# omkhairate/MetalPathtracer

Measured on AMD Instinct MI355X. Metric: Mrays/s at 1920x1080x256spp on scene.xml, higher is better.
Workload: dtype f32; 1 GPU; scene.xml 1920x1080 x 256 spp per step, depth 8 (181 steps timed); prims=4971, bvh_nodes=2289, bvh_builder=device, rng=philox4x32-10 (pixel,sample,bounce), pipeline=wave-local wavefront, reference-order walk, parallelism=8x8-tile interleave over 1 rank(s), rays=161154900585

## Files before the change

### metalpathtracer_amd/csrc/mpt_device.h

```cpp
#pragma once
#include <hip/hip_runtime.h>
#include <stdint.h>

#define MPT_WAVE 64
#define MPT_NSHARD 16
#define MPT_NGROUP 8
#define MPT_NONE 0xFFFFFFFFu

struct F3 {
    float x, y, z;
};
__device__ __forceinline__ F3 f3(float x, float y, float z) { return F3{x, y, z}; }
__device__ __forceinline__ F3 operator+(F3 a, F3 b) { return F3{a.x + b.x, a.y + b.y, a.z + b.z}; }
__device__ __forceinline__ F3 operator-(F3 a, F3 b) { return F3{a.x - b.x, a.y - b.y, a.z - b.z}; }
__device__ __forceinline__ F3 operator*(F3 a, float s) { return F3{a.x * s, a.y * s, a.z * s}; }
__device__ __forceinline__ F3 operator*(float s, F3 a) { return F3{s * a.x, s * a.y, s * a.z}; }
__device__ __forceinline__ F3 operator-(F3 a) { return F3{-a.x, -a.y, -a.z}; }
__device__ __forceinline__ float dot3(F3 a, F3 b) { return a.x * b.x + a.y * b.y + a.z * b.z; }
__device__ __forceinline__ F3 cross3(F3 a, F3 b) {
    return F3{a.y * b.z - a.z * b.y, a.z * b.x - a.x * b.z, a.x * b.y - a.y * b.x};
}
#ifndef MPT_FAST_RCP
#define MPT_FAST_RCP 3
#endif
#define MPT_RCP_LO 1.1754943508222875e-38f
#define MPT_RCP_HI 8.5070591730234616e+37f
__device__ __forceinline__ float rcp_chain(float x) {
    float r = __builtin_amdgcn_rcpf(x);
    const float e0 = fmaf(-x, r, 1.0f);
    r = fmaf(e0, r, r);
    float q = r;
    const float e1 = fmaf(-x, q, 1.0f);
    q = fmaf(e1, r, q);
    const float e2 = fmaf(-x, q, 1.0f);
    return fmaf(e2, r, q);
}
__device__ __forceinline__ bool rcp_chain_exact(float x) { return fabsf(x) >= MPT_RCP_LO && fabsf(x) <= MPT_RCP_HI; }
__device__ __forceinline__ float mpt_rcp(float x) {
#if MPT_FAST_RCP == 2
    return rcp_chain(x);
#elif MPT_FAST_RCP == 3
    if (__builtin_expect(__ballot(!rcp_chain_exact(x)) == 0ull, 1)) return rcp_chain(x);
    return 1.0f / x;
#elif MPT_FAST_RCP == 1
    float r = rcp_chain(x);
    if (__builtin_expect(!rcp_chain_exact(x), 0)) r = 1.0f / x;
    return r;
#else
    return 1.0f / x;
#endif
}
__device__ __forceinline__ void mpt_rcp3(float x, float y, float z, float& ix, float& iy, float& iz) {
#if MPT_FAST_RCP == 3
    if (__builtin_expect(__ballot(!(rcp_chain_exact(x) && rcp_chain_exact(y) && rcp_chain_exact(z))) == 0ull, 1)) {
        ix = rcp_chain(x);
        iy = rcp_chain(y);
        iz = rcp_chain(z);
        return;
    }
    ix = 1.0f / x;
    iy = 1.0f / y;
    iz = 1.0f / z;
#else
    ix = mpt_rcp(x);
    iy = mpt_rcp(y);
    iz = mpt_rcp(z);
#endif
}
__device__ __forceinline__ F3 normalize3(F3 a) {
    float inv = mpt_rcp(sqrtf(dot3(a, a)));
    return a * inv;
}
#ifndef MPT_LEAN_SQRT
#define MPT_LEAN_SQRT 1
#endif
#define MPT_SQRT_LO 0x1p-96f
#define MPT_NORM_HI 0x1p126f
__device__ __forceinline__ float sqrt_core(float x) {
    const float s = __builtin_amdgcn_sqrtf(x);
    const float lo = __uint_as_float(__float_as_uint(s) - 1u), hi = __uint_as_float(__float_as_uint(s) + 1u);
    const float vlo = fmaf(-lo, s, x), vhi = fmaf(-hi, s, x);
    float r = vlo <= 0.0f ? lo : s;
    r = vhi > 0.0f ? hi : r;
    return r;
}
__device__ __forceinline__ bool sqrt_core_exact(float x) { return x >= MPT_SQRT_LO && x < INFINITY; }
__device__ __forceinline__ bool norm_core_exact(float l2) { return l2 >= MPT_SQRT_LO && l2 <= MPT_NORM_HI; }
__device__ __forceinline__ float inv_len_core(float l2) { return rcp_chain(sqrt_core(l2)); }
template <bool LEAN>
__device__ __forceinline__ F3 normalize3(F3 a) {
    if (LEAN && MPT_LEAN_SQRT) {
        const float l2 = dot3(a, a);
        if (__builtin_expect(__ballot(!norm_core_exact(l2)) == 0ull, 1)) return a * inv_len_core(l2);
        return a * mpt_rcp(sqrtf(l2));
    }
    return normalize3(a);
}
#ifndef MPT_LEAN_CDIV
#define MPT_LEAN_CDIV 1
#endif
__device__ __forceinline__ float cdiv_recip(float W) {
    const float r0 = __builtin_amdgcn_rcpf(W);
    const float e = fmaf(-W, r0, 1.0f);
    return fmaf(e, r0, r0);
}
__device__ __forceinline__ float cdiv_chain(float x, float W, float r) {
    float q = x * r;
    const float e1 = fmaf(-W, q, x);
    q = fmaf(e1, r, q);
    const float e2 = fmaf(-W, q, x);
    return fmaf(e2, r, q);
}
__device__ __forceinline__ float clamp01(float v) { return fminf(fmaxf(v, 0.0f), 1.0f); }

__device__ __forceinline__ uint32_t pcg_hash(uint32_t s) {
    uint32_t state = s * 747796405u + 2891336453u;
    uint32_t word = ((state >> ((state >> 28u) + 4u)) ^ state);
    return (word >> 22u) ^ word;
}
__device__ __forceinline__ float pcg_float(uint32_t s) { return (float)pcg_hash(s) / 4294967296.0f; }

struct U4 {
    uint32_t x, y, z, w;
};
template <bool UNIFORM_KEY = false>
__device__ __forceinline__ U4 philox4x32_10(uint32_t c0, uint32_t c1, uint32_t c2, uint32_t c3, uint32_t k0,
                                            uint32_t k1) {
#pragma unroll
    for (int r = 0; r < 10; ++r) {
        uint64_t p0 = (uint64_t)0xD2511F53u * c0;
        uint64_t p1 = (uint64_t)0xCD9E8D57u * c2;
        uint32_t n0 = (uint32_t)(p1 >> 32) ^ c1 ^ k0;
        uint32_t n1 = (uint32_t)p1;
        uint32_t n2 = (uint32_t)(p0 >> 32) ^ c3 ^ k1;
        uint32_t n3 = (uint32_t)p0;
        c0 = n0; c1 = n1; c2 = n2; c3 = n3;
        k0 += 0x9E3779B9u;
        k1 += 0xBB67AE85u;
        if (UNIFORM_KEY) asm volatile("" : "+s"(k0), "+s"(k1));
    }
    return U4{c0, c1, c2, c3};
}
__device__ __forceinline__ float u01(uint32_t x) { return (float)(x >> 8) * 5.9604644775390625e-08f; }

__device__ __forceinline__ void sincos_2pi(float u, float& s_out, float& c_out) {
    float x = u * 4.0f;
    int q = (int)(x + 0.5f);
    float r = x - (float)q;
    float th = r * 1.57079637050628662109375f;
    float t2 = th * th;
    float ps = -1.98412701138295233249664306640625e-4f + t2 * 2.755731884462875314056873321533203125e-6f;
    ps = 8.3333337679505348205566406250e-3f + t2 * ps;
    ps = -0.16666667163372039794921875f + t2 * ps;
    float s = th + (th * t2) * ps;
    float pc = -1.38888892251998186111450195312500e-3f + t2 * 2.48015876422869041562080383300781250e-5f;
// ... 56 lines not shown
struct WorkCount {
    uint32_t node_visits, aabb_hits, prim_tests;
    uint32_t node_iters, prim_iters, outer_iters;
#ifdef MPT_DEBUG_WAVE_TIMES
    unsigned long long t_box, t_leaf;
    uint32_t wait_leaf, wait_done;
#endif
#ifdef MPT_OT_TIMES
    unsigned long long ot_node_cycles, ot_leaf_cycles, ot_node_trips, ot_leaf_trips, ot_rounds;
    unsigned long long ot_node_lanes, ot_leaf_lanes;
    unsigned long long ot_lds_nodes, ot_glb_nodes, ot_lds_prims, ot_glb_prims;
    unsigned long long ot_pops, ot_pop_iters, ot_pop_calls, ot_pop_wave_iters;
#endif
};
#ifdef MPT_DEBUG_WAVE_TIMES
#define MPT_TIC(var) unsigned long long var = __builtin_amdgcn_s_memtime()
#define MPT_TOC(acc, var)                                          \
    do {                                                           \
        unsigned long long now_ = __builtin_amdgcn_s_memtime();    \
        (acc) += now_ - (var);                                     \
        (var) = now_;                                              \
    } while (0)
#else
#define MPT_TIC(var) do { } while (0)
#define MPT_TOC(acc, var) do { } while (0)
#endif

struct Prim3 {
    float4 p0, p1, p2;
};
#ifndef MPT_LEAN_INT24
#define MPT_LEAN_INT24 1
#endif
typedef const __attribute__((address_space(3))) char* LdsBytes;
__device__ __forceinline__ uint32_t mul_u24(uint32_t a, uint32_t b) { return (uint32_t)__umul24(a, b); }
#ifndef MPT_LEAN_CAMSPHERE
#define MPT_LEAN_CAMSPHERE 1
#endif
__device__ __forceinline__ void sphere_cam_terms(F3 o, float4 p0, float4& p1, float4& p2) {
    const F3 oc = o - f3(p0.x, p0.y, p0.z);
    const float radius = p1.x;
    p1.z = dot3(oc, oc) - radius * radius;
    p2.x = oc.x;
    p2.y = oc.y;
    p2.z = oc.z;
}
template <bool LEAN = false, bool PRIMARY = false>
__device__ __forceinline__ Prim3 load_prim(const SceneDev& sc, LdsNodes lds, uint32_t i, F3 o = F3{0.0f, 0.0f, 0.0f}) {
    Prim3 r;
    if (LEAN && MPT_LEAN_INT24) {
        const uint32_t off = mul_u24(i, 48u);
        if (i < sc.n_lds_prims) {
            const LdsNodes q = (LdsNodes)((LdsBytes)lds + (sc.lds_prim_off * 16u + off));
            const v4f a = q[0], b = q[1], c = q[2];
            r.p0 = make_float4(a.x, a.y, a.z, a.w);
            r.p1 = make_float4(b.x, b.y, b.z, b.w);
            r.p2 = make_float4(c.x, c.y, c.z, c.w);
        } else {
            const float4* q = (const float4*)((const char*)sc.prims + off);
            r.p0 = q[0];
            r.p1 = q[1];
            r.p2 = q[2];
            if (MPT_LEAN_CAMSPHERE && PRIMARY && prim_type(r.p0) == 0) sphere_cam_terms(o, r.p0, r.p1, r.p2);
        }
        return r;
    }
    if (i < sc.n_lds_prims) {
        const LdsNodes q = lds + sc.lds_prim_off + 3u * i;
        const v4f a = q[0], b = q[1], c = q[2];
        r.p0 = make_float4(a.x, a.y, a.z, a.w);
        r.p1 = make_float4(b.x, b.y, b.z, b.w);
        r.p2 = make_float4(c.x, c.y, c.z, c.w);
    } else {
        r.p0 = sc.prims[3 * i];
        r.p1 = sc.prims[3 * i + 1];
        r.p2 = sc.prims[3 * i + 2];
    }
    return r;
}

template <bool COUNT, bool LEAN = false, bool PRIMARY = false>
__device__ __forceinline__ void leaf_test(const SceneDev& sc, LdsNodes lds, uint32_t first, uint32_t count, F3 o, F3 d,
                                          float& best_t, int& best_prim, WorkCount& wc) {
    constexpr bool cam_terms = LEAN && MPT_LEAN_INT24 && MPT_LEAN_CAMSPHERE && PRIMARY;
    for (uint32_t k = 0; k < count; ++k) {
        const Prim3 pr = load_prim<LEAN, cam_terms>(sc, lds, first + k, o);
        const float4 p0 = pr.p0, p1 = pr.p1, p2 = pr.p2;
        if (COUNT) {
            wc.prim_tests++;
            if (first_active_lane()) wc.prim_iters++;
        }
        const int ptype = prim_type(p0);
        if (ptype == 1) {
            F3 v0 = f3(p0.x, p0.y, p0.z), e1 = f3(p1.x, p1.y, p1.z), e2 = f3(p2.x, p2.y, p2.z);
            F3 h = cross3(d, e2);
            float a = dot3(e1, h);
            if (fabsf(a) > 1e-5f) {
                float f = mpt_rcp(a);
                F3 s = o - v0;
                float u = f * dot3(s, h);
                if (u >= 0.0f && u <= 1.0f) {
                    F3 q = cross3(s, e1);
                    float v = f * dot3(d, q);
                    if (v >= 0.0f && u + v <= 1.0f) {
                        float tt = f * dot3(e2, q);
                        if (tt > 0.0001f && tt < best_t) {
                            best_t = tt;
                            best_prim = (int)(first + k);
                        }
                    }
                }
            }
        } else if (ptype == 0) {
            F3 c = f3(p0.x, p0.y, p0.z);
            float radius = p1.x;
            const F3 oc = cam_terms ? f3(p2.x, p2.y, p2.z) : o - c;
            float a = dot3(d, d);
            float b = dot3(oc, d);
            const float cc = cam_terms ? p1.z : dot3(oc, oc) - radius * radius;
            const float disc = b * b - a * cc;
            if (!(b >= 0.0f) && disc > 0.0f) {
                const float sq = sqrtf(disc);
                const float temp = (-b - sq) / a;
                const bool closer = temp < best_t && temp > 0.0001f;
                best_t = closer ? temp : best_t;
                best_prim = closer ? (int)(first + k) : best_prim;
            }
        }
    }
}


#ifndef MPT_LEAF_EARLY
#define MPT_LEAF_EARLY 8u
#endif
#define MPT_NODE_HOLD 0x80000000u
#ifndef MPT_LEAN_ONECMP
#define MPT_LEAN_ONECMP 1
#endif
__device__ __forceinline__ bool slab_hit(float4 n0, float4 n1, F3 o, float idx, float idy, float idz, float best_t) {
    float t0 = (n0.x - o.x) * idx, t1 = (n1.x - o.x) * idx;
    float lo = fmaxf(0.0001f, idx < 0.0f ? t1 : t0);
    float hi = fminf(best_t, idx < 0.0f ? t0 : t1);
    t0 = (n0.y - o.y) * idy;
    t1 = (n1.y - o.y) * idy;
    lo = fmaxf(lo, idy < 0.0f ? t1 : t0);
    hi = fminf(hi, idy < 0.0f ? t0 : t1);
    t0 = (n0.z - o.z) * idz;
    t1 = (n1.z - o.z) * idz;
    lo = fmaxf(lo, idz < 0.0f ? t1 : t0);
    hi = fminf(hi, idz < 0.0f ? t0 : t1);
    return hi > lo;
}
template <bool COUNT, bool ALL_LDS, bool BUDGETED, bool LEAN = false, bool PRIMARY = false>
__device__ __forceinline__ bool closest_hit_resume(const SceneDev& sc, LdsNodes lds_nodes, F3 o, F3 d, uint32_t& node,
                                                   float& best_t, int& best_prim, uint32_t budget, WorkCount& wc,
                                                   uint32_t min_active = 0u) {
    float idx, idy, idz;
    mpt_rcp3(d.x, d.y, d.z, idx, idy, idz);
    const uint32_t n_nodes = sc.n_nodes, n_lds = sc.n_lds_nodes;
    uint32_t i = (d.x != d.x || d.y != d.y || d.z != d.z) ? n_nodes : node;
    uint32_t trips = 0;
    MPT_TIC(tic_);
    for (;;) {
        uint32_t skip = 0;
        unsigned long long search_mask = __ballot(i < n_nodes);
        const uint32_t n_entered0 = (uint32_t)__popcll(search_mask), n_entered = max(n_entered0, 1u);
#ifdef MPT_DEBUG_WAVE_TIMES
        uint32_t my_trips = 0, round_trips = 0;
#endif
        uint32_t n_searching = n_entered0;
        while (n_searching * MPT_LEAF_EARLY >= n_entered && (!BUDGETED || trips < budget)) {
            const bool searching = LEAN && MPT_LEAN_ONECMP ? __builtin_amdgcn_inverse_ballot_w64(search_mask) : i < n_nodes;
#ifdef MPT_DEBUG_WAVE_TIMES
            my_trips += searching ? 1u : 0u;
            round_trips++;
#endif
            const uint32_t j = LEAN && MPT_LEAN_ONECMP ? i : (i < n_nodes - 1u ? i : n_nodes - 1u);
            float4 n0 = make_float4(0, 0, 0, 0), n1 = n0;
            bool box = false;
            if (searching) {
                if (ALL_LDS || j < n_lds) {
                    const v4f a = lds_nodes[2 * j], b = lds_nodes[2 * j + 1];
                    n0 = make_float4(a.x, a.y, a.z, a.w);
                    n1 = make_float4(b.x, b.y, b.z, b.w);
                } else {
                    n0 = sc.nodes[2 * j];
                    n1 = sc.nodes[2 * j + 1];
                }
                box = slab_hit(n0, n1, o, idx, idy, idz, best_t);
            }
            const uint32_t A = __float_as_uint(n0.w), B = __float_as_uint(n1.w);
            if (COUNT) {
                wc.node_visits += searching ? 1u : 0u;
                wc.aabb_hits += (searching && box) ? 1u : 0u;
                if (first_active_lane()) wc.node_iters++;
            }
            const uint32_t next = box ? A : B;
            i = searching ? next : i;
            skip = searching ? B : skip;
            if (BUDGETED) trips++;
            search_mask = __ballot(i < n_nodes);
            n_searching = (uint32_t)__popcll(search_mask);
        }
#ifdef MPT_DEBUG_WAVE_TIMES
        if (COUNT) {
            if ((i & MPT_NODE_HOLD) != 0u) wc.wait_leaf += round_trips - my_trips;
            else wc.wait_done += round_trips - my_trips;
        }
#endif
        MPT_TOC(wc.t_box, tic_);
        if ((i & MPT_NODE_HOLD) != 0u) {
            const uint32_t enc = i & ~MPT_NODE_HOLD;
            if (COUNT && first_active_lane()) wc.outer_iters++;
            leaf_test<COUNT, LEAN, PRIMARY>(sc, lds_nodes, enc >> 4, (enc & 15u) + 1u, o, d, best_t, best_prim, wc);
            i = skip;
        }
        MPT_TOC(wc.t_leaf, tic_);
        if (BUDGETED && trips >= budget) break;
        const unsigned long long going = __ballot(i < n_nodes);
        if (going == 0ull) break;
        if (BUDGETED && (uint32_t)__popcll(going) < min_active) break;
    }
    node = i;
    return i >= n_nodes;
}

template <bool COUNT, bool ALL_LDS>
__device__ __forceinline__ void closest_hit(const SceneDev& sc, LdsNodes lds_nodes, F3 o, F3 d,
                                            float& best_t, int& best_prim, WorkCount& wc) {
    uint32_t node = 0;
    best_t = INFINITY;
    best_prim = -1;
    closest_hit_resume<COUNT, ALL_LDS, false>(sc, lds_nodes, o, d, node, best_t, best_prim, 0xFFFFFFFFu, wc);
}

struct HitInfo {
    F3 point, normal;
    bool front;
    int mat;
    int orig_id;
};
template <bool LEAN = false>
__device__ __forceinline__ HitInfo finish_hit(const SceneDev& sc, LdsNodes lds, F3 o, F3 d, float t, int prim) {
    HitInfo h;
    const Prim3 pr = load_prim<LEAN>(sc, lds, (uint32_t)prim);
    const float4 p0 = pr.p0, p1 = pr.p1, p2 = pr.p2;
    h.point = o + t * d;
    if (prim_type(p0) == 1) {
        h.normal = normalize3<LEAN>(cross3(f3(p1.x, p1.y, p1.z), f3(p2.x, p2.y, p2.z)));
    } else {
        h.normal = normalize3<LEAN>(h.point - f3(p0.x, p0.y, p0.z));
    }
    h.mat = __float_as_int(p1.w);
    h.orig_id = __float_as_int(p2.w);
    h.front = dot3(h.normal, d) < 0.0f;
    if (!h.front) h.normal = -h.normal;
    return h;
}

struct PathState {
    F3 o, d;
    F3 thr;
    F3 L;
    float La;
    uint32_t path;
    uint32_t bounce;
};

struct ShadeParams {
    int rng_mode, bsdf_mode, max_depth;
    uint32_t seed_lo, seed_hi;
    uint32_t primitive_count;
};

struct PathRngDev {
    uint32_t pixel, sample;
    uint32_t lit_seed;
};

struct BounceRandoms {
    float uz, uphi, u_extra;
};
template <bool LEAN = false>
__device__ __forceinline__ BounceRandoms draw_bounce_randoms(const ShadeParams& sp, const PathRngDev& g, uint32_t bounce) {
    BounceRandoms b;
    if (!LEAN && sp.rng_mode == 0) {
        b.uz = b.uphi = b.u_extra = pcg_float(g.lit_seed);
    } else {
        const U4 r = philox4x32_10<true>(g.pixel, g.sample, bounce, 0u, sp.seed_lo, sp.seed_hi);
        b.uz = u01(r.x);
        b.uphi = u01(r.y);
        b.u_extra = u01(r.z);
    }
    return b;
}
template <bool LEAN = false>
__device__ __forceinline__ F3 random_unit_vector(const ShadeParams& sp, const BounceRandoms& b) {
    float z = 2.0f * b.uz - 1.0f, s, c;
    if (!LEAN && sp.rng_mode == 0) {
        const float t = 2.0f * 3.14159274101257324f * b.uphi;
        s = sinf(t);
        c = cosf(t);
    } else {
        sincos_2pi(b.uphi, s, c);
    }
    const float rr = sqrtf(1.0f - z * z);
    return f3(rr * c, rr * s, z);
}

__device__ __forceinline__ F3 reflect3(F3 i, F3 n) { return i - 2.0f * dot3(n, i) * n; }
__device__ __forceinline__ F3 refract3(F3 i, F3 n, float eta) {
    float dd = dot3(n, i);
    float k = 1.0f - eta * eta * (1.0f - dd * dd);
    if (k < 0.0f) return f3(0, 0, 0);
    return eta * i - (eta * dd + sqrtf(k)) * n;
}
__device__ __forceinline__ bool mirror_angle(float ri, F3 normal, F3 rayDir, float u) {
    float cosT = dot3(-1.0f * rayDir, normal);
    float sinT = sqrtf(1.0f - cosT * cosT);
    float r0 = (1.0f - ri) / (1.0f + ri);
    r0 = r0 * r0;
    float m = 1.0f - cosT;
    float m2 = m * m;
    float refl = r0 + (1.0f - r0) * (m2 * m2 * m);
    return (ri * sinT > 1.0f) || (refl > u);
}

template <bool LEAN = false>
__device__ __forceinline__ bool shade_bounce(const SceneDev& sc, LdsNodes lds, const ShadeParams& sp, const PathRngDev& g,
                                             PathState& ps, float t, int prim) {
    if (prim < 0) {
        F3 ud = normalize3<LEAN>(ps.d);
        float tt = 0.5f * (ud.y + 1.0f);
        F3 sky = f3(1.0f + (0.6f - 1.0f) * tt, 1.0f + (0.7f - 1.0f) * tt, 1.0f + (1.0f - 1.0f) * tt);
        ps.L.x += ps.thr.x * sky.x;
        ps.L.y += ps.thr.y * sky.y;
        ps.L.z += ps.thr.z * sky.z;
        ps.La += 1.0f;
        return false;
    }
    const BounceRandoms rnd = draw_bounce_randoms<LEAN>(sp, g, ps.bounce);
    HitInfo h = finish_hit<LEAN>(sc, lds, ps.o, ps.d, t, prim);
    if ((uint32_t)h.orig_id >= sp.primitive_count) return false;
    float4 m0, m1;
    if ((uint32_t)h.mat < sc.n_lds_mats) {
        const LdsNodes q = lds + sc.lds_mat_off + 2u * (uint32_t)h.mat;
        const v4f a = q[0], b = q[1];
        m0 = make_float4(a.x, a.y, a.z, a.w);
        m1 = make_float4(b.x, b.y, b.z, b.w);
    } else {
        m0 = sc.mats[2 * h.mat];
        m1 = sc.mats[2 * h.mat + 1];
    }
    const float mtype = m0.w, power = m1.w;
    if (power > 0.0f || mtype == 2.0f) {
        ps.L.x += ps.thr.x * m1.x * power;
        ps.L.y += ps.thr.y * m1.y * power;
        ps.L.z += ps.thr.z * m1.z * power;
        ps.La += power;
    }
    const float u_extra = rnd.u_extra;
    F3 ruv = random_unit_vector<LEAN>(sp, rnd);
    F3 nd;
    bool through = false;
    if (LEAN) {
        nd = normalize3<LEAN>(h.normal + ruv);
    } else if (sp.bsdf_mode == 2 && mtype == 0.0f) {
        F3 c;
        if (sp.rng_mode == 0) {
            uint32_t s = g.lit_seed;
            c.x = pcg_float(s) * 2.0f - 1.0f;
            s = pcg_hash(s);
            c.y = pcg_float(s) * 2.0f - 1.0f;
            s = pcg_hash(s);
            c.z = pcg_float(s) * 2.0f - 1.0f;
// ... 23 lines not shown
```

### metalpathtracer_amd/csrc/mpt_kernels.h

```cpp
#pragma once
#include <hip/hip_runtime.h>
#include <stdint.h>

#include "mpt_device.h"
#include "mpt_wl_lean.h"
#include "mpt_lean_entry.h"

#ifndef MPT_MIN_WAVES
#define MPT_MIN_WAVES 8
#endif

struct QueueDev {
    float4* od;
    float4* dt;
    float4* tl;
    uint2* ia;
};

struct PassDesc {
    uint32_t in_count[MPT_NSHARD];
    uint32_t item_prefix[MPT_NSHARD + 1];
    uint32_t n_items;
    uint32_t regen_base;
    uint32_t range_end[MPT_NGROUP];
// ... 452 lines not shown
#define MPT_WL_RING 512u
#define MPT_LDS_MATS_N 32u
#define MPT_LDS_CFG_F4 16u
__host__ __device__ __forceinline__ uint32_t mpt_lds_cfg_off_f4(uint32_t lds_mat_off) { return lds_mat_off + 2u * MPT_LDS_MATS_N; }
__host__ __device__ __forceinline__ uint32_t mpt_lds_image_end_f4(uint32_t lds_mat_off) { return mpt_lds_cfg_off_f4(lds_mat_off) + MPT_LDS_CFG_F4; }
#define MPT_WL_BLOCK 1024u
#define MPT_WL_NO_BUDGET 0x7FFFFFFFu
#define MPT_RING_HAS_LIGHT 0x100u
struct WaveRings {
    float4* base;
    uint32_t n;
    __host__ __device__ float4* od() const { return base; }
    __host__ __device__ float4* dt() const { return base + n; }
    __host__ __device__ float4* tl() const { return base + 2u * (size_t)n; }
    __host__ __device__ uint4* ia() const { return (uint4*)(base + 3u * (size_t)n); }
    __host__ __device__ uint4* tv() const { return (uint4*)(base + 4u * (size_t)n); }
};
__device__ __forceinline__ bool ring_has_light(const PathState& ps) {
    return (__float_as_uint(ps.L.x) | __float_as_uint(ps.L.y) | __float_as_uint(ps.L.z) | __float_as_uint(ps.La)) != 0u;
}
__device__ __forceinline__ uint32_t sample_of_path(const PassParams& pp, uint32_t path) {
    const uint32_t chunk = path >> 6;
    return pp.sample_begin + (pp.s_shift != 0xFFu ? chunk & (pp.S - 1u) : chunk % pp.S);
}
__device__ __forceinline__ void ring_push(const WaveRings& ring, uint32_t at, const PathState& ps, const PathRngDev& g) {
    ring.od()[at] = make_float4(ps.o.x, ps.o.y, ps.o.z, ps.d.x);
    ring.dt()[at] = make_float4(ps.d.y, ps.d.z, ps.thr.x, ps.thr.y);
    const bool lit = ring_has_light(ps);
    ring.ia()[at] = make_uint4(__float_as_uint(ps.thr.z), ps.path, g.pixel, ps.bounce | (lit ? MPT_RING_HAS_LIGHT : 0u));
    if (lit) ring.tl()[at] = make_float4(ps.L.x, ps.L.y, ps.L.z, ps.La);
}
__device__ __forceinline__ void ring_pop(const PassParams& pp, const WaveRings& ring, uint32_t at, PathState& ps, PathRngDev& g) {
    const float4 a = ring.od()[at], b = ring.dt()[at];
    const uint4 ia = ring.ia()[at];
    ps.o = f3(a.x, a.y, a.z);
    ps.d = f3(a.w, b.x, b.y);
    ps.thr = f3(b.z, b.w, __uint_as_float(ia.x));
    ps.path = ia.y;
    g.pixel = ia.z;
    ps.bounce = ia.w & 0xFFu;
    g.sample = sample_of_path(pp, ps.path);
    ps.L = f3(0.0f, 0.0f, 0.0f);
    ps.La = 0.0f;
    if ((ia.w & MPT_RING_HAS_LIGHT) != 0u) {
        const float4 cc = ring.tl()[at];
        ps.L = f3(cc.x, cc.y, cc.z);
        ps.La = cc.w;
    }
    g.lit_seed = 0;
    if (pp.sp.rng_mode == 0) g.lit_seed = pcg_hash(pcg_hash(pp.pixel_seed[g.pixel]));
}
__device__ __forceinline__ void ring_push_hit(const WaveRings& ring, uint32_t at, const PathState& ps, float t, uint32_t prim) {
    ring.od()[at] = make_float4(ps.o.x, ps.o.y, ps.o.z, ps.d.x);
    ring.dt()[at] = make_float4(ps.d.y, ps.d.z, ps.thr.x, ps.thr.y);
    const bool lit = ring_has_light(ps);
    ring.ia()[at] = make_uint4(__float_as_uint(ps.thr.z), ps.path, (__float_as_uint(t) & 0x7FFFFFFFu) | (lit ? 0x80000000u : 0u),
                               (prim & 0x07FFFFFFu) | (ps.bounce << 27));
    if (lit) ring.tl()[at] = make_float4(ps.L.x, ps.L.y, ps.L.z, ps.La);
}
__device__ __forceinline__ void ring_pop_hit(const WaveRings& ring, uint32_t at, PathState& ps, float& t, int& prim) {
    const float4 a = ring.od()[at], b = ring.dt()[at];
    const uint4 ia = ring.ia()[at];
    ps.o = f3(a.x, a.y, a.z);
    ps.d = f3(a.w, b.x, b.y);
    ps.thr = f3(b.z, b.w, __uint_as_float(ia.x));
    ps.path = ia.y;
    t = __uint_as_float(ia.z & 0x7FFFFFFFu);
    prim = (int)(ia.w & 0x07FFFFFFu);
    ps.bounce = ia.w >> 27;
    ps.L = f3(0.0f, 0.0f, 0.0f);
    ps.La = 0.0f;
    if ((ia.z & 0x80000000u) != 0u) {
        const float4 cc = ring.tl()[at];
        ps.L = f3(cc.x, cc.y, cc.z);
        ps.La = cc.w;
    }
}

struct WaveBudgets {
    uint32_t b[MPT_WL_LEVELS];
    uint32_t min_active[MPT_WL_LEVELS];
};

#ifndef MPT_WL_THREADS_N
#define MPT_WL_THREADS_N 768
#endif
#ifndef MPT_WL_WAVES_N
#define MPT_WL_WAVES_N 6
#endif
#ifndef MPT_WL_CARRY
#define MPT_WL_CARRY 1
#endif
#if MPT_WL_CARRY && defined(MPT_WL_FIFO)
#error "MPT_WL_CARRY needs ring 0 to be a stack: build MPT_WL_FIFO with -DMPT_WL_CARRY=0"
#endif
#define MPT_WL_THREADS(ALL_LDS) MPT_WL_THREADS_N
#define MPT_WL_WAVES(ALL_LDS) MPT_WL_WAVES_N
template <bool COUNT, bool ALL_LDS, bool LEAN = false>
__device__ __forceinline__ void wavelocal_body(const PassParams& pp, const WaveRings& ring, const WaveBudgets& budgets, uint32_t wl_block, uint32_t wl_min,
                                               uint32_t wl_div, const WlLean& lean = WlLean{0u, 0u, 0u});
template <bool COUNT, bool ALL_LDS>
__global__ __launch_bounds__(MPT_WL_THREADS(ALL_LDS), MPT_WL_WAVES(ALL_LDS)) void k_wavelocal(PassParams pp, WaveRings ring, WaveBudgets budgets,
                                                                                             uint32_t wl_block, uint32_t wl_min, uint32_t wl_div) {
    wavelocal_body<COUNT, ALL_LDS>(pp, ring, budgets, wl_block, wl_min, wl_div);
}
#ifndef MPT_WL_CORUN_SGPRS
#define MPT_WL_CORUN_SGPRS 96
#endif
template <bool ALL_LDS>
__global__ __launch_bounds__(MPT_WL_THREADS(ALL_LDS), MPT_WL_WAVES(ALL_LDS)) __attribute__((amdgpu_num_sgpr(MPT_WL_CORUN_SGPRS)))
void k_wavelocal_corun(PassParams pp, WaveRings ring, WaveBudgets budgets, uint32_t wl_block, uint32_t wl_min, uint32_t wl_div) {
    wavelocal_body<false, ALL_LDS>(pp, ring, budgets, wl_block, wl_min, wl_div);
}
template <bool ALL_LDS>
__global__ __launch_bounds__(MPT_WL_THREADS(ALL_LDS), MPT_WL_WAVES(ALL_LDS)) void k_wavelocal_lean(PassParams pp, WaveRings ring, WaveBudgets budgets,
                                                                                                  uint32_t wl_block, uint32_t wl_min, uint32_t wl_div, WlLean lean) {
    wavelocal_body<false, ALL_LDS, true>(pp, ring, budgets, wl_block, wl_min, wl_div, lean);
}
template <bool ALL_LDS>
__global__ __launch_bounds__(MPT_WL_THREADS(ALL_LDS), MPT_WL_WAVES(ALL_LDS)) __attribute__((amdgpu_num_sgpr(MPT_WL_CORUN_SGPRS)))
void k_wavelocal_lean_corun(PassParams pp, WaveRings ring, WaveBudgets budgets, uint32_t wl_block, uint32_t wl_min, uint32_t wl_div, WlLean lean) {
    wavelocal_body<false, ALL_LDS, true>(pp, ring, budgets, wl_block, wl_min, wl_div, lean);
}
template <bool COUNT, bool ALL_LDS, bool LEAN>
__device__ __forceinline__ void wavelocal_body(const PassParams& pp, const WaveRings& ring, const WaveBudgets& budgets, uint32_t wl_block, uint32_t wl_min,
                                               uint32_t wl_div, const WlLean& lean) {
    static_assert(!(LEAN && COUNT), "the lean body does not count");
    extern __shared__ float4 lds_nodes_raw[];
    const uint32_t cfg_off = mpt_lds_cfg_off_f4(pp.scene.lds_mat_off);
    if (threadIdx.x == 0) {
        announce_resident(pp);
        lds_nodes_raw[cfg_off + 0] = make_float4(pp.cam.x, pp.cam.y, pp.cam.z, pp.W);
        lds_nodes_raw[cfg_off + 1] = make_float4(pp.first.x, pp.first.y, pp.first.z, pp.H);
        lds_nodes_raw[cfg_off + 2] = make_float4(pp.vu.x, pp.vu.y, pp.vu.z, LEAN && MPT_LEAN_CDIV ? cdiv_recip(pp.W) : 0.0f);
        lds_nodes_raw[cfg_off + 3] = make_float4(pp.vv.x, pp.vv.y, pp.vv.z, LEAN && MPT_LEAN_CDIV ? cdiv_recip(pp.H) : 0.0f);
        uint32_t* w = (uint32_t*)(lds_nodes_raw + cfg_off + 4);
        for (uint32_t k = 0; k < MPT_WL_LEVELS; ++k) {
            w[k] = budgets.b[k];
            w[8u + k] = budgets.min_active[k];
        }
        static_assert(4u * (10u - 4u) >= 22u && MPT_LDS_CFG_F4 >= 12u, "configuration block too small");
        w[16] = wl_block;
        w[17] = wl_min;
        w[18] = wl_div * (((uint32_t)(gridDim.x * (blockDim.x >> 6)) + MPT_NGROUP - 1u) / MPT_NGROUP);
        w[19] = pp.desc->total_paths / (pp.S * 64u);
        if (LEAN) {
            w[20] = lean.s_mul;
            w[21] = lean.s_shift;
        }
        if (LEAN && MPT_LEAN_ENTRY) {
            const float4 none = make_float4(0.0f, 0.0f, 0.0f, 0.0f);
            const bool tree = pp.scene.n_nodes != 0u;
            const LeanEntry e = lean_entry_terms(tree ? pp.scene.nodes[0] : none, tree ? pp.scene.nodes[1] : none, pp.scene.n_nodes, pp.cam.x, pp.cam.y, pp.cam.z);
            lds_nodes_raw[cfg_off + 10] = make_float4(e.ilo[0], e.ilo[1], e.ilo[2], __uint_as_float(e.entry));
            lds_nodes_raw[cfg_off + 11] = make_float4(e.ihi[0], e.ihi[1], e.ihi[2], __uint_as_float(e.entry_primary));
        }
    }
    if (LEAN && MPT_LEAN_CAMSPHERE) stage_nodes_lean(pp.scene, lds_nodes_raw, pp.cam);
    else stage_nodes(pp.scene, lds_nodes_raw);
    MPT_CLOCK_BEGIN();
    const LdsNodes lds_nodes = (LdsNodes)lds_nodes_raw;
    const __attribute__((address_space(3))) uint32_t* lds_cfg_u32 = (const __attribute__((address_space(3))) uint32_t*)(lds_nodes + cfg_off + 4u);
    const uint32_t lane = threadIdx.x & 63u;
    const uint32_t wave_id = blockIdx.x * (blockDim.x >> 6) + (threadIdx.x >> 6);
#ifdef MPT_DEBUG_WAVE_TIMES
    const uint32_t n_waves = gridDim.x * (blockDim.x >> 6);
#endif
    const uint32_t wbase = wave_id * (MPT_WL_LEVELS * MPT_WL_RING);
    const uint32_t M = MPT_WL_RING - 1u;
    uint32_t head[MPT_WL_LEVELS], cnt[MPT_WL_LEVELS];
#pragma unroll
    for (uint32_t k = 0; k < MPT_WL_LEVELS; ++k) head[k] = cnt[k] = 0;
    uint32_t cur = 0, end = 0;
    uint32_t grp = blockIdx.x & (MPT_NGROUP - 1u);
    uint32_t seen = 0;
    bool exhausted = false;
    uint32_t tile_cached = 0xFFFFFFFFu, tile_xy_cached = 0u;
    float uvx_cached = 0.0f, uvy_cached = 0.0f;
    uint32_t n_rays = 0, n_paths = 0;
    WorkCount wc = {};
#if MPT_WL_CARRY
    bool kept = false;
    PathState ps = {};
    float best_t = INFINITY;
    int best_prim = -1;
#endif
#ifdef MPT_DEBUG_WAVE_TIMES
    const unsigned long long t_start = __builtin_amdgcn_s_memrealtime();
    unsigned long long t_exh = 0ull, t_claim = 0ull, dbg_steps = 0ull, dbg_left = 0ull, dbg_blk = 0ull;
    unsigned long long reg_select = 0, reg_fetch = 0, reg_trace = 0, reg_shade = 0, reg_push = 0;
#endif
    for (;;) {
        MPT_TIC(tic_);
        int level = -1;
#if MPT_WL_CARRY
        const unsigned long long carry = __ballot(kept);
        if (cnt[0] + (uint32_t)__popcll(carry) >= 64u) level = 0;
#pragma unroll
        for (int k = (int)MPT_WL_LEVELS - 1; k >= 1; --k)
            if (level <= 0 && cnt[k] >= 64u) level = k;
#else
#pragma unroll
        for (int k = (int)MPT_WL_LEVELS - 1; k >= 0; --k)
            if (level < 0 && cnt[k] >= 64u) level = k;
#endif
        if (level < 0) {
            if (!exhausted && cur == end) {
                uint32_t k = 0, blk = 0, rend = 0;
                bool got = false;
                if (lane == 0) {
                    const uint32_t c_block = lds_cfg_u32[16], c_min = lds_cfg_u32[17], c_div = lds_cfg_u32[18], c_tiles = lds_cfg_u32[19];
                    for (uint32_t t = 0; t < MPT_NGROUP && !got; ++t) {
                        const uint32_t re = range_paths(c_tiles, pp.S, grp);
                        const uint32_t left = seen < re ? re - seen : 0u;
                        blk = (left / c_div) & ~63u;
                        blk = blk < c_min ? c_min : (blk > c_block ? c_block : blk);
                        if (t > 0u) blk = c_min;
                        k = atomicAdd(&pp.ctr[MPT_CTR_CURSOR(grp)], blk);
                        if (k < re) {
                            got = true;
                            rend = re;
                        } else {
                            grp = (grp + 1u) & (MPT_NGROUP - 1u);
                            seen = 0;
                        }
                    }
                }
                got = __builtin_amdgcn_readfirstlane((int)got) != 0;
                k = __builtin_amdgcn_readfirstlane(k);
                blk = __builtin_amdgcn_readfirstlane(blk);
                rend = __builtin_amdgcn_readfirstlane(rend);
                grp = __builtin_amdgcn_readfirstlane(grp);
                seen = k;
#ifdef MPT_DEBUG_WAVE_TIMES
                if (got) {
                    t_claim = __builtin_amdgcn_s_memrealtime();
                    dbg_steps = 0ull;
                    dbg_blk = blk;
                } else {
                    t_exh = __builtin_amdgcn_s_memrealtime();
                    for (uint32_t q = 0; q < MPT_WL_LEVELS; ++q) dbg_left |= (unsigned long long)cnt[q] << (12u * q);
                }
#endif
                if (!got) {
                    exhausted = true;
                } else {
                    cur = k;
                    end = (k + blk < rend) ? k + blk : rend;
                }
            }
            if (exhausted) {
                uint32_t total = 0;
#pragma unroll
                for (int k = 0; k < (int)MPT_WL_LEVELS; ++k) total += cnt[k];
                if (total == 0u) break;
                level = (int)MPT_WL_LEVELS;
            }
        }
#ifdef MPT_DEBUG_WAVE_TIMES
        if (!exhausted) dbg_steps += 1ull << (12u * (uint32_t)(level + 1));
#endif
        MPT_TOC(reg_select, tic_);
#if MPT_WL_CARRY
        float hit_t = __uint_as_float(__float_as_uint(best_t) & 0x7FFFFFFFu);
        int hit_prim = (int)((uint32_t)best_prim & 0x07FFFFFFu);
        ps.bounce &= 31u;
        best_t = INFINITY;
        best_prim = -1;
#else
        PathState ps;
        float best_t = INFINITY;
        int best_prim = -1;
        float hit_t = 0.0f;
        int hit_prim = -1;
#endif
        PathRngDev g;
        bool valid = false;
        uint32_t node = 0;
        uint32_t budget = 0xFFFFFFFFu, min_active = 0u;
        bool fresh = false;
        bool need_shade = false;
        if (level < 0) {
            fresh = true;
            const uint32_t pchunk = range_chunk_to_path_chunk(pp, cur >> 6, grp);
            cur += 64u;
            uint32_t tl, sidx;
            if (pp.s_shift != 0xFFu) {
                tl = pchunk >> pp.s_shift;
                sidx = pchunk & (pp.S - 1u);
            } else {
                tl = pchunk / pp.S;
                sidx = pchunk - tl * pp.S;
            }
            const bool new_tile = tl != tile_cached;
            if (new_tile) {
                tile_cached = tl;
                if (LEAN) {
                    const uint32_t T = tl * pp.nranks + pp.rank, ty = (T * lean.tile_mul) >> MPT_WL_LEAN_TILE_SHIFT;
                    tile_xy_cached = (T - ty * pp.tiles_x) | (ty << 16);
                } else {
                    tile_xy_cached = (uint32_t)__builtin_amdgcn_readfirstlane((int)pp.tile_xy[tl]);
                }
            }
            PathState np;
            np.path = pchunk * 64u + lane;
            const uint32_t px = (tile_xy_cached & 0xFFFFu) * 8u + (lane & 7u), py = (tile_xy_cached >> 16) * 8u + (lane >> 3);
            CamView cv;
            {
                const v4f c0 = lds_nodes[cfg_off], c1 = lds_nodes[cfg_off + 1u], c2 = lds_nodes[cfg_off + 2u], c3 = lds_nodes[cfg_off + 3u];
                cv.cam = f3(c0.x, c0.y, c0.z);
                cv.first = f3(c1.x, c1.y, c1.z);
                cv.vu = f3(c2.x, c2.y, c2.z);
                cv.vv = f3(c3.x, c3.y, c3.z);
                cv.W = c0.w;
                cv.H = c1.w;
                cv.rW = c2.w;
                cv.rH = c3.w;
            }
            if (new_tile) pixel_uv(cv, px, py, uvx_cached, uvy_cached);
            if (px < pp.width && py < pp.height) {
                gen_primary<LEAN>(pp, cv, px, py, uvx_cached, uvy_cached, pp.sample_begin + sidx, np, g);
                valid = true;
            }
            n_paths += (uint32_t)__popcll(__ballot(valid));
            ps = np;
        } else {
            uint32_t my_ring = 0, my_off = 0;
            bool take = false;
            uint32_t assigned = 0;
#if MPT_WL_CARRY
            const uint32_t slot = wave_rank(~carry), room = 64u - (uint32_t)__popcll(carry);
            const bool empty = !kept;
#else
            const uint32_t slot = lane, room = 64u;
            const bool empty = true;
#endif
#pragma unroll
            for (int k = (int)MPT_WL_LEVELS - 1; k >= 0; --k) {
                const bool use = (level == (int)MPT_WL_LEVELS) || (level == k);
                uint32_t tk = use ? cnt[k] : 0u;
                tk = tk < room - assigned ? tk : room - assigned;
                if (empty && slot >= assigned && slot < assigned + tk) {
                    take = true;
                    my_ring = (uint32_t)k;
#ifdef MPT_WL_FIFO
                    my_off = (head[k] + (slot - assigned)) & M;
#else
                    my_off = cnt[k] - tk + (slot - assigned);
#endif
                }
                (void)k;
#ifdef MPT_WL_FIFO
                head[k] = (head[k] + tk) & M;
#endif
                cnt[k] -= tk;
                assigned += tk;
            }
            if (level < (int)MPT_WL_LEVELS) {
                budget = (uint32_t)__builtin_amdgcn_readfirstlane((int)lds_cfg_u32[level]);
                min_active = (uint32_t)__builtin_amdgcn_readfirstlane((int)lds_cfg_u32[8 + level]);
            }
            if (level == (int)MPT_WL_LEVELS && assigned >= 12u) min_active = assigned / 3u;
            if (take) {
                const uint32_t at = wbase + my_ring * MPT_WL_RING + my_off;
                uint4 tv = make_uint4(0u, 0u, 0u, 0u);
                if (my_ring > 0u) tv = ring.tv()[at];
                ring_pop_hit(ring, at, ps, hit_t, hit_prim);
                need_shade = my_ring == 0u;
                if (my_ring > 0u) {
                    node = tv.x;
                    best_t = __uint_as_float(tv.y);
                    best_prim = (int)tv.z;
                } else {
                    fresh = true;
                }
                valid = true;
            }
#if MPT_WL_CARRY
            if (kept) {
                need_shade = true;
                fresh = true;
                valid = true;
            }
#endif
        }
        if (need_shade) {
            uint32_t px, py, sidx;
            path_to_pixel<LEAN>(pp, ps.path, px, py, sidx, lean.tile_mul, (LdsWords)lds_cfg_u32);
            g.pixel = LEAN && MPT_LEAN_INT24 ? mul_u24(py, pp.width) + px : py * pp.width + px;
            g.sample = pp.sample_begin + sidx;
            g.lit_seed = 0;
            if (!LEAN && pp.sp.rng_mode == 0) g.lit_seed = pcg_hash(pcg_hash(pp.pixel_seed[g.pixel]));
            if (!shade_bounce<LEAN>(pp.scene, lds_nodes, pp.sp, g, ps, hit_t, hit_prim)) {
                store_slot(pp.slots, ps.path, clamp01(ps.L.x), clamp01(ps.L.y), clamp01(ps.L.z), clamp01(ps.La));
                valid = false;
            }
        }
        if (LEAN && MPT_LEAN_ENTRY && fresh) {
            const bool d_ok = fmaxf(fmaxf(fabsf(ps.d.x), fabsf(ps.d.y)), fabsf(ps.d.z)) <= MPT_LEAN_ENTRY_DMAX;
            if (level < 0) {
                const uint32_t entry_primary = ((const __attribute__((address_space(3))) uint32_t*)(lds_nodes + cfg_off + 11u))[3];
                node = d_ok ? entry_primary : 0u;
            } else {
                const v4f elo = lds_nodes[cfg_off + 10u], ehi = lds_nodes[cfg_off + 11u];
                const bool in = elo.x <= ps.o.x && ps.o.x <= ehi.x && elo.y <= ps.o.y && ps.o.y <= ehi.y && elo.z <= ps.o.z && ps.o.z <= ehi.z;
                node = in && d_ok ? __float_as_uint(elo.w) : 0u;
            }
        }
        const bool budgeted = level >= 0 && (level < (int)MPT_WL_LEVELS || min_active != 0u) &&
                              ((level < (int)MPT_WL_LEVELS - 1 && budget < MPT_WL_NO_BUDGET) || min_active != 0u);
        const int park_ring = level + 1 < (int)MPT_WL_LEVELS ? level + 1 : (int)MPT_WL_LEVELS - 1;
        bool alive = false, parked = false;
        MPT_TOC(reg_fetch, tic_);
#ifdef MPT_DEBUG_WAVE_TIMES
        const WorkCount wc0 = wc;
#endif
        n_rays += (uint32_t)__popcll(__ballot(valid && fresh));
        if (valid) {
            bool done;
            if (budgeted)
                done = closest_hit_resume<COUNT, ALL_LDS, true, LEAN>(pp.scene, lds_nodes, ps.o, ps.d, node, best_t, best_prim,
                                                                     budget, wc, min_active);
            else if (LEAN && MPT_LEAN_CAMSPHERE && level < 0)
                done = closest_hit_resume<COUNT, ALL_LDS, false, LEAN, true>(pp.scene, lds_nodes, ps.o, ps.d, node, best_t, best_prim,
                                                                            0xFFFFFFFFu, wc);
            else
                done = closest_hit_resume<COUNT, ALL_LDS, false, LEAN>(pp.scene, lds_nodes, ps.o, ps.d, node, best_t, best_prim,
                                                                      0xFFFFFFFFu, wc);
            MPT_TOC(reg_trace, tic_);
#ifdef MPT_DEBUG_WAVE_TIMES
            if (COUNT) {
                unsigned long long* lv = (unsigned long long*)(ring.tv() + (size_t)n_waves * MPT_WL_LEVELS * MPT_WL_RING) +
                                         16ull * n_waves + 8ull * (unsigned)(level + 1);
                if (first_active_lane()) atomicAdd(lv + 0, 1ull);
                if (wc.node_iters != wc0.node_iters) atomicAdd(lv + 1, (unsigned long long)(wc.node_iters - wc0.node_iters));
                if (wc.prim_iters != wc0.prim_iters) atomicAdd(lv + 3, (unsigned long long)(wc.prim_iters - wc0.prim_iters));
                atomicAdd(lv + 2, (unsigned long long)(wc.node_visits - wc0.node_visits));
                atomicAdd(lv + 4, (unsigned long long)(wc.prim_tests - wc0.prim_tests));
                atomicAdd(lv + 5, 1ull);
                if (wc.wait_leaf != wc0.wait_leaf) atomicAdd(lv + 7, (unsigned long long)(wc.wait_leaf - wc0.wait_leaf));
                if (done) atomicAdd(lv + 6, 1ull);
            }
#endif
            if (done) {
                alive = best_prim >= 0;
                if (!alive) {
                    shade_bounce<LEAN>(pp.scene, lds_nodes, pp.sp, g, ps, best_t, -1);
                    store_slot(pp.slots, ps.path, clamp01(ps.L.x), clamp01(ps.L.y), clamp01(ps.L.z), clamp01(ps.La));
                }
            } else {
                parked = true;
            }
        }
        MPT_TOC(reg_shade, tic_);
        const unsigned long long am = __ballot(alive), pm = __ballot(parked);
        if (pm != 0ull) {
            uint32_t h = 0, c = 0;
#pragma unroll
            for (int k = 1; k < (int)MPT_WL_LEVELS; ++k)
                if (k == park_ring) {
                    h = head[k];
                    c = cnt[k];
                }
            if (parked) {
                const uint32_t at = wbase + (uint32_t)park_ring * MPT_WL_RING + ((h + c + wave_rank(pm)) & M);
                ring_push_hit(ring, at, ps, 0.0f, 0u);
                ring.tv()[at] = make_uint4(node, __float_as_uint(best_t), (uint32_t)best_prim, 0u);
            }
#pragma unroll
            for (int k = 1; k < (int)MPT_WL_LEVELS; ++k)
                if (k == park_ring) cnt[k] = c + (uint32_t)__popcll(pm);
        }
#if MPT_WL_CARRY
        bool keep = cnt[0] + (uint32_t)__popcll(am) >= 64u;
#pragma unroll
        for (int k = 1; k < (int)MPT_WL_LEVELS; ++k) keep = keep && cnt[k] < 64u;
        kept = keep && alive;
#else
        const bool keep = false;
#endif
#ifdef MPT_DEBUG_WAVE_TIMES
        if (COUNT && (am | pm) != 0ull) {
            unsigned long long* rt = (unsigned long long*)(ring.tv() + (size_t)n_waves * MPT_WL_LEVELS * MPT_WL_RING) + 16ull * n_waves + 8ull * 14ull;
            const unsigned long long lit_a = __ballot(alive && ring_has_light(ps)), lit_p = __ballot(parked && ring_has_light(ps));
            if (lane == 0u) {
                if (am != 0ull) {
                    atomicAdd(rt + 8 + (keep ? 0 : 1), (unsigned long long)__popcll(am));
                    atomicAdd(rt + 8 + (keep ? 2 : 3), (unsigned long long)__popcll(lit_a));
                    atomicAdd(rt + 8 + (keep ? 4 : 5), 1ull);
                }
                if (pm != 0ull) {
                    atomicAdd(rt + 0, (unsigned long long)__popcll(pm));
                    atomicAdd(rt + 1, (unsigned long long)__popcll(lit_p));
                    atomicAdd(rt + 2, 1ull);
                }
            }
        }
#endif
        if (am != 0ull && !keep) {
            if (alive) {
                const uint32_t at = wbase + ((head[0] + cnt[0] + wave_rank(am)) & M);
                ring_push_hit(ring, at, ps, best_t, (uint32_t)best_prim);
            }
            cnt[0] += (uint32_t)__popcll(am);
        }
        uint32_t worst = 0;
#pragma unroll
        for (uint32_t k = 0; k < MPT_WL_LEVELS; ++k) worst = cnt[k] > worst ? cnt[k] : worst;
        if (worst > MPT_WL_RING) pp.desc->overflow = 1u;
        MPT_TOC(reg_push, tic_);
    }
#ifdef MPT_DEBUG_WAVE_TIMES
    if (lane == 0) {
        unsigned long long* dbg = (unsigned long long*)(ring.tv() + (size_t)n_waves * MPT_WL_LEVELS * MPT_WL_RING);
        dbg[8 * wave_id] = t_start;
        dbg[8 * wave_id + 1] = t_exh;
        dbg[8 * wave_id + 2] = __builtin_amdgcn_s_memrealtime();
        dbg[8 * wave_id + 3] = t_claim;
        dbg[8 * wave_id + 4] = dbg_steps;
        dbg[8 * wave_id + 5] = dbg_left;
        dbg[8 * wave_id + 6] = dbg_blk;
        unsigned long long* reg = dbg + 8ull * n_waves + 8ull * wave_id;
        reg[0] = reg_select;
        reg[1] = reg_fetch;
        reg[2] = reg_trace;
        reg[3] = reg_shade;
        reg[4] = reg_push;
        reg[5] = wc.t_box;
        reg[6] = wc.t_leaf;
    }
#endif
    MPT_CLOCK_END();
    flush_stats<COUNT>(pp.desc, lane == 0u ? n_rays : 0u, lane == 0u ? n_paths : 0u, wc);
    note_wave_exit(pp);
}

__global__ __launch_bounds__(256, 8) void k_resolve_sum(PassParams pp, float4* sum, uint32_t n_local_tiles) {
    const uint32_t n = n_local_tiles * 64u;
    for (uint32_t i = blockIdx.x * blockDim.x + threadIdx.x; i < n; i += gridDim.x * blockDim.x) {
        const uint32_t tl = i >> 6, lane = i & 63u;
        uint32_t px, py, s0;
        if (!path_to_pixel(pp, (tl * pp.S) * 64u + lane, px, py, s0)) continue;
        float4 acc = sum[py * pp.width + px];
        const uint32_t base = tl * pp.S;
        uint32_t s = 0;
        for (; s + 4u <= pp.S; s += 4u) {
            const float4 v0 = load_slot(pp.slots, (base + s) * 64u + lane), v1 = load_slot(pp.slots, (base + s + 1u) * 64u + lane),
                         v2 = load_slot(pp.slots, (base + s + 2u) * 64u + lane), v3 = load_slot(pp.slots, (base + s + 3u) * 64u + lane);
            acc.x += v0.x; acc.y += v0.y; acc.z += v0.z; acc.w += v0.w;
            acc.x += v1.x; acc.y += v1.y; acc.z += v1.z; acc.w += v1.w;
            acc.x += v2.x; acc.y += v2.y; acc.z += v2.z; acc.w += v2.w;
            acc.x += v3.x; acc.y += v3.y; acc.z += v3.z; acc.w += v3.w;
        }
        for (; s < pp.S; ++s) {
            const float4 v = load_slot(pp.slots, (base + s) * 64u + lane);
            acc.x += v.x; acc.y += v.y; acc.z += v.z; acc.w += v.w;
        }
        sum[py * pp.width + px] = acc;
    }
}

__device__ __forceinline__ void add_moments(float4& m, const float4& v) {
    const float l = (0.2126f * v.x + 0.7152f * v.y) + 0.0722f * v.z;
    m.x += v.x * v.x; m.y += v.y * v.y; m.z += v.z * v.z; m.w += l * l;
}
__global__ __launch_bounds__(256, 8) void k_resolve_sum_moments(PassParams pp, float4* sum, float4* m2, uint32_t n_local_tiles) {
    const uint32_t n = n_local_tiles * 64u;
    for (uint32_t i = blockIdx.x * blockDim.x + threadIdx.x; i < n; i += gridDim.x * blockDim.x) {
        const uint32_t tl = i >> 6, lane = i & 63u;
        uint32_t px, py, s0;
        if (!path_to_pixel(pp, (tl * pp.S) * 64u + lane, px, py, s0)) continue;
        float4 acc = sum[py * pp.width + px];
        float4 m = m2[py * pp.width + px];
        const uint32_t base = tl * pp.S;
        uint32_t s = 0;
        for (; s + 4u <= pp.S; s += 4u) {
            const float4 v0 = load_slot(pp.slots, (base + s) * 64u + lane), v1 = load_slot(pp.slots, (base + s + 1u) * 64u + lane),
                         v2 = load_slot(pp.slots, (base + s + 2u) * 64u + lane), v3 = load_slot(pp.slots, (base + s + 3u) * 64u + lane);
            acc.x += v0.x; acc.y += v0.y; acc.z += v0.z; acc.w += v0.w;
            acc.x += v1.x; acc.y += v1.y; acc.z += v1.z; acc.w += v1.w;
            acc.x += v2.x; acc.y += v2.y; acc.z += v2.z; acc.w += v2.w;
// ... 129 lines not shown
```

### metalpathtracer_amd/csrc/mpt_lean_entry.h

```cpp
#pragma once
#include <stdint.h>

#ifndef MPT_LEAN_ENTRY
#define MPT_LEAN_ENTRY 1
#endif
#define MPT_LEAN_ENTRY_M 0x1p-10f
#define MPT_LEAN_ENTRY_DMAX 2.0f
#if defined(__HIPCC__)
#define MPT_LEAN_ENTRY_HD __host__ __device__
#else
#define MPT_LEAN_ENTRY_HD
#endif

struct LeanEntry {
    float ilo[3], ihi[3];
    uint32_t entry;
    uint32_t entry_primary;
};

template <class V4>
MPT_LEAN_ENTRY_HD inline LeanEntry lean_entry_terms(const V4& n0, const V4& n1, uint32_t n_nodes, float cam_x, float cam_y, float cam_z) {
    const float m = MPT_LEAN_ENTRY_M, inf = __builtin_huge_valf();
    const float lo[3] = {n0.x, n0.y, n0.z}, hi[3] = {n1.x, n1.y, n1.z}, cam[3] = {cam_x, cam_y, cam_z};
    uint32_t A0;
    const float a0 = n0.w;
    __builtin_memcpy(&A0, &a0, sizeof A0);
    LeanEntry e;
    bool on = A0 != 0u && A0 < n_nodes, cam_in = true;
    for (int a = 0; a < 3; ++a) {
        e.ilo[a] = lo[a] + 2.0f * m;
        e.ihi[a] = hi[a] - 2.0f * m;
        on = on && (lo[a] - e.ilo[a] <= -m) && (hi[a] - e.ihi[a] >= m) && e.ilo[a] <= e.ihi[a];
        cam_in = cam_in && e.ilo[a] <= cam[a] && cam[a] <= e.ihi[a];
    }
    if (!on)
        for (int a = 0; a < 3; ++a) {
            e.ilo[a] = inf;
            e.ihi[a] = -inf;
        }
    e.entry = on ? A0 : 0u;
    e.entry_primary = on && cam_in ? A0 : 0u;
    return e;
}
```

Baseline: 62470 Mrays/s.

## Special-case the final BVH tail leaf with a wave-uniform containment test

Finds the last leaf on the root's skip chain (the tail node) and rewrites every LDS skip link that points to it into a tail marker. The traversal loop then exits at that marker and handles the tail leaf outside the loop, using a precomputed box-containment test on the ray origin, with a slab test as fallback only when some lane needs it. The aim is to take the last-leaf visit out of the divergent traversal loop and run it with a wave-uniform leaf index. In exchange it adds per-block setup work (a scan over the LDS links plus a barrier), extra config slots, and depends on subtle assumptions about tree link encoding.

```diff
diff --git a/metalpathtracer_amd/csrc/mpt_device.h b/metalpathtracer_amd/csrc/mpt_device.h
--- a/metalpathtracer_amd/csrc/mpt_device.h
+++ b/metalpathtracer_amd/csrc/mpt_device.h
@@ -1,6 +1,8 @@
 #pragma once
 #include <hip/hip_runtime.h>
 #include <stdint.h>
+
+#include "mpt_lean_entry.h"
 
 #define MPT_WAVE 64
 #define MPT_NSHARD 16
@@ -363,10 +365,11 @@
     hi = fminf(hi, idz < 0.0f ? t0 : t1);
     return hi > lo;
 }
+static_assert(MPT_LEAN_LEAF_BIT == MPT_NODE_HOLD && MPT_NODE_TAIL < MPT_NODE_HOLD, "mpt_lean_entry.h: the leaf bit and the tail marker");
 template <bool COUNT, bool ALL_LDS, bool BUDGETED, bool LEAN = false, bool PRIMARY = false>
 __device__ __forceinline__ bool closest_hit_resume(const SceneDev& sc, LdsNodes lds_nodes, F3 o, F3 d, uint32_t& node,
                                                    float& best_t, int& best_prim, uint32_t budget, WorkCount& wc,
-                                                   uint32_t min_active = 0u) {
+                                                   uint32_t min_active = 0u, LdsNodes tail_cfg = nullptr) {
     float idx, idy, idz;
     mpt_rcp3(d.x, d.y, d.z, idx, idy, idz);
     const uint32_t n_nodes = sc.n_nodes, n_lds = sc.n_lds_nodes;
@@ -433,6 +436,34 @@
         if (going == 0ull) break;
         if (BUDGETED && (uint32_t)__popcll(going) < min_active) break;
     }
+    if (LEAN && ALL_LDS && MPT_LEAN_ENTRY && MPT_LEAN_TAIL) {
+        if (i == MPT_NODE_TAIL) {
+            const bool d_ok = fmaxf(fmaxf(fabsf(d.x), fabsf(d.y)), fabsf(d.z)) <= MPT_LEAN_ENTRY_DMAX;
+            bool hit;
+            uint32_t leaf;
+            if (PRIMARY) {
+                const __attribute__((address_space(3))) uint32_t* w = (const __attribute__((address_space(3))) uint32_t*)tail_cfg;
+                leaf = w[3];
+                hit = d_ok && w[7] != 0u;
+            } else {
+                const v4f tlo = tail_cfg[0], thi = tail_cfg[1];
+                leaf = __float_as_uint(tlo.w);
+                hit = d_ok && tlo.x <= o.x && o.x <= thi.x && tlo.y <= o.y && o.y <= thi.y && tlo.z <= o.z && o.z <= thi.z;
+            }
+#if !defined(MPT_LEAN_TAIL_NO_SLAB)
+            if (__ballot(!hit) != 0ull) {
+                if (!hit) {
+                    const v4f a = tail_cfg[2], b = tail_cfg[3];
+                    hit = slab_hit(make_float4(a.x, a.y, a.z, a.w), make_float4(b.x, b.y, b.z, b.w), o, idx, idy, idz, best_t);
+                }
+            }
+#endif
+            if (hit) {
+                const uint32_t enc = (uint32_t)__builtin_amdgcn_readfirstlane((int)leaf) & ~MPT_NODE_HOLD;
+                leaf_test<COUNT, LEAN, PRIMARY>(sc, lds_nodes, enc >> 4, (enc & 15u) + 1u, o, d, best_t, best_prim, wc);
+            }
+        }
+    }
     node = i;
     return i >= n_nodes;
 }
diff --git a/metalpathtracer_amd/csrc/mpt_kernels.h b/metalpathtracer_amd/csrc/mpt_kernels.h
--- a/metalpathtracer_amd/csrc/mpt_kernels.h
+++ b/metalpathtracer_amd/csrc/mpt_kernels.h
@@ -628,12 +628,38 @@
             const float4 none = make_float4(0.0f, 0.0f, 0.0f, 0.0f);
             const bool tree = pp.scene.n_nodes != 0u;
             const LeanEntry e = lean_entry_terms(tree ? pp.scene.nodes[0] : none, tree ? pp.scene.nodes[1] : none, pp.scene.n_nodes, pp.cam.x, pp.cam.y, pp.cam.z);
-            lds_nodes_raw[cfg_off + 10] = make_float4(e.ilo[0], e.ilo[1], e.ilo[2], __uint_as_float(e.entry));
-            lds_nodes_raw[cfg_off + 11] = make_float4(e.ihi[0], e.ihi[1], e.ihi[2], __uint_as_float(e.entry_primary));
+            uint32_t entry = e.entry, entry_primary = e.entry_primary;
+            if (ALL_LDS && MPT_LEAN_TAIL) {
+                static_assert(MPT_LDS_CFG_F4 >= 16u, "configuration block too small");
+                const LeanTail t = lean_tail_terms(pp.scene.nodes, pp.scene.n_nodes, pp.cam.x, pp.cam.y, pp.cam.z);
+                lds_nodes_raw[cfg_off + 12] = make_float4(t.tlo[0], t.tlo[1], t.tlo[2], __uint_as_float(t.leaf));
+                lds_nodes_raw[cfg_off + 13] = make_float4(t.thi[0], t.thi[1], t.thi[2], __uint_as_float(t.tail_primary));
+                float4 t0 = make_float4(0.0f, 0.0f, 0.0f, 0.0f), t1 = t0;
+                if (t.node != 0u) {
+                    t0 = pp.scene.nodes[2u * t.node];
+                    t1 = pp.scene.nodes[2u * t.node + 1u];
+                }
+                t1.w = __uint_as_float(t.node);
+                lds_nodes_raw[cfg_off + 14] = t0;
+                lds_nodes_raw[cfg_off + 15] = t1;
+                if (t.node != 0u && entry == t.node) entry = MPT_NODE_TAIL;
+                if (t.node != 0u && entry_primary == t.node) entry_primary = MPT_NODE_TAIL;
+            }
+            lds_nodes_raw[cfg_off + 10] = make_float4(e.ilo[0], e.ilo[1], e.ilo[2], __uint_as_float(entry));
+            lds_nodes_raw[cfg_off + 11] = make_float4(e.ihi[0], e.ihi[1], e.ihi[2], __uint_as_float(entry_primary));
         }
     }
     if (LEAN && MPT_LEAN_CAMSPHERE) stage_nodes_lean(pp.scene, lds_nodes_raw, pp.cam);
     else stage_nodes(pp.scene, lds_nodes_raw);
+    if (LEAN && ALL_LDS && MPT_LEAN_ENTRY && MPT_LEAN_TAIL) {
+        const uint32_t tail_node = __float_as_uint(lds_nodes_raw[cfg_off + 15].w);
+        if (tail_node != 0u) {
+            uint32_t* links = (uint32_t*)lds_nodes_raw;
+            for (uint32_t k = threadIdx.x; k < pp.scene.n_lds_nodes * 2u; k += blockDim.x)
+                if (links[4u * k + 3u] == tail_node) links[4u * k + 3u] = MPT_NODE_TAIL;
+        }
+        __syncthreads();
+    }
     MPT_CLOCK_BEGIN();
     const LdsNodes lds_nodes = (LdsNodes)lds_nodes_raw;
     const __attribute__((address_space(3))) uint32_t* lds_cfg_u32 = (const __attribute__((address_space(3))) uint32_t*)(lds_nodes + cfg_off + 4u);
@@ -896,13 +922,13 @@
             bool done;
             if (budgeted)
                 done = closest_hit_resume<COUNT, ALL_LDS, true, LEAN>(pp.scene, lds_nodes, ps.o, ps.d, node, best_t, best_prim,
-                                                                     budget, wc, min_active);
+                                                                     budget, wc, min_active, lds_nodes + cfg_off + 12u);
             else if (LEAN && MPT_LEAN_CAMSPHERE && level < 0)
                 done = closest_hit_resume<COUNT, ALL_LDS, false, LEAN, true>(pp.scene, lds_nodes, ps.o, ps.d, node, best_t, best_prim,
-                                                                            0xFFFFFFFFu, wc);
+                                                                            0xFFFFFFFFu, wc, 0u, lds_nodes + cfg_off + 12u);
             else
                 done = closest_hit_resume<COUNT, ALL_LDS, false, LEAN>(pp.scene, lds_nodes, ps.o, ps.d, node, best_t, best_prim,
-                                                                      0xFFFFFFFFu, wc);
+                                                                      0xFFFFFFFFu, wc, 0u, lds_nodes + cfg_off + 12u);
             MPT_TOC(reg_trace, tic_);
 #ifdef MPT_DEBUG_WAVE_TIMES
             if (COUNT) {
diff --git a/metalpathtracer_amd/csrc/mpt_lean_entry.h b/metalpathtracer_amd/csrc/mpt_lean_entry.h
--- a/metalpathtracer_amd/csrc/mpt_lean_entry.h
+++ b/metalpathtracer_amd/csrc/mpt_lean_entry.h
@@ -42,3 +42,62 @@
     e.entry_primary = on && cam_in ? A0 : 0u;
     return e;
 }
+
+#ifndef MPT_LEAN_TAIL
+#define MPT_LEAN_TAIL 1
+#endif
+#define MPT_NODE_TAIL 0x40000000u
+#define MPT_LEAN_LEAF_BIT 0x80000000u
+
+struct LeanTail {
+    float tlo[3], thi[3];
+    uint32_t node;
+    uint32_t leaf;
+    uint32_t tail_primary;
+};
+
+template <class V4>
+MPT_LEAN_ENTRY_HD inline LeanTail lean_tail_terms(const V4* nodes, uint32_t n_nodes, float cam_x, float cam_y, float cam_z) {
+    const float m = MPT_LEAN_ENTRY_M, inf = __builtin_huge_valf();
+    const float cam[3] = {cam_x, cam_y, cam_z};
+    LeanTail t;
+    for (int a = 0; a < 3; ++a) {
+        t.tlo[a] = inf;
+        t.thi[a] = -inf;
+    }
+    t.node = t.leaf = t.tail_primary = 0u;
+    if (n_nodes == 0u || n_nodes >= MPT_NODE_TAIL) return t;
+    uint32_t T, B, steps = 0u;
+    const float a0 = nodes[0].w;
+    __builtin_memcpy(&T, &a0, sizeof T);
+    if (T == 0u || T >= n_nodes) return t;
+    for (;; ++steps) {
+        const float b = nodes[2u * T + 1u].w;
+        __builtin_memcpy(&B, &b, sizeof B);
+        if (B >= n_nodes) break;
+        if (B == 0u || steps == n_nodes) return t;
+        T = B;
+    }
+    uint32_t leaf;
+    const float l = nodes[2u * T].w;
+    __builtin_memcpy(&leaf, &l, sizeof leaf);
+    if ((leaf & MPT_LEAN_LEAF_BIT) == 0u) return t;
+    const float lo[3] = {nodes[2u * T].x, nodes[2u * T].y, nodes[2u * T].z}, hi[3] = {nodes[2u * T + 1u].x, nodes[2u * T + 1u].y, nodes[2u * T + 1u].z};
+    float tlo[3], thi[3];
+    bool on = true, cam_in = true;
+    for (int a = 0; a < 3; ++a) {
+        tlo[a] = lo[a] + 2.0f * m;
+        thi[a] = hi[a] - 2.0f * m;
+        on = on && (lo[a] - tlo[a] <= -m) && (hi[a] - thi[a] >= m) && tlo[a] <= thi[a];
+        cam_in = cam_in && tlo[a] <= cam[a] && cam[a] <= thi[a];
+    }
+    if (!on) return t;
+    for (int a = 0; a < 3; ++a) {
+        t.tlo[a] = tlo[a];
+        t.thi[a] = thi[a];
+    }
+    t.node = T;
+    t.leaf = leaf;
+    t.tail_primary = cam_in ? 1u : 0u;
+    return t;
+}
```

Measured after the change: 64160 Mrays/s (median of 6 runs). 1.03x the previous value.
